# aquaskyline/Clairvoyante

Measured on AMD Instinct MI355X. Metric: candidate tensors/sec, higher is better.
Workload: dtype f32

## Files before the change

clairvoyante_amd/csrc/cv_pileup.hip:

```cpp
#include <hip/hip_runtime.h>
#include <hipcub/hipcub.hpp>

#include <cstdarg>
#include <cstdio>
#include <cstdlib>
#include <cstring>
#include <algorithm>
#include <new>
#include <string>
#include <thread>
#include <vector>

#include "../../include/clairvoyante_amd.h"
#include "cv_draw_core.hpp"

void cv_set_error(const char *fmt, ...);

#define PL_HIP(expr)                                                                              \
    do {                                                                                          \
        hipError_t _e = (expr);                                                                   \
        if (_e != hipSuccess) {                                                                   \
            cv_set_error("%s failed: %s (%s:%d)", #expr, hipGetErrorString(_e), __FILE__, __LINE__); \
            return 1;                                                                             \
        }                                                                                         \
// ... 25 lines not shown
    return ch == 'A' ? 0 : ch == 'C' ? 1 : ch == 'G' ? 2 : ch == 'T' ? 3 : -1;
}

__global__ void rebase_q0(seg_t *__restrict__ segs, int64_t n, uint32_t base)
{
    int64_t t = (int64_t)blockIdx.x * blockDim.x + threadIdx.x;
    if (t < n) segs[t].q0 += base;
}

__global__ void bucket_build(const int32_t *__restrict__ cands, int n, int32_t lo, int64_t nb,
                             int32_t *__restrict__ first)
{
    int64_t b = (int64_t)blockIdx.x * blockDim.x + threadIdx.x;
    if (b >= nb) return;
    int64_t target = (int64_t)lo + (b << BUCKET_SHIFT);
    int l = 0, h = n;
    while (l < h) {
        int m = (l + h) >> 1;
        if ((int64_t)cands[m] < target) l = m + 1; else h = m;
    }
    first[b] = l;
}

constexpr int SC_SEGS = 512;
constexpr int SC_CANDS = 40;

__global__ void __launch_bounds__(1024)
pileup_scatter(const seg_t *__restrict__ segs, int64_t nseg, const uint8_t *__restrict__ seq,
               const uint8_t *__restrict__ ref, int64_t ref_first, int64_t ref_len,
               const int32_t *__restrict__ cands, int n, const int32_t *__restrict__ bucket_first,
               int32_t bucket_lo, int64_t nb, int32_t *__restrict__ cnt, uint8_t *__restrict__ touched, int left)
{
    __shared__ int32_t tab[SC_CANDS * WIDTH * NCNT];
    const int64_t s0 = (int64_t)blockIdx.x * SC_SEGS;
    const int64_t s1 = s0 + SC_SEGS < nseg ? s0 + SC_SEGS : nseg;
    for (int k = threadIdx.x; k < SC_CANDS * WIDTH * NCNT; k += blockDim.x) tab[k] = 0;
    int i0;
    {
        const int64_t lo_c = (int64_t)segs[s0].pos - FLANK;
        int64_t b = (lo_c - bucket_lo) >> BUCKET_SHIFT;
        if (b < 0) b = 0;
        if (b >= nb) b = nb - 1;
        i0 = bucket_first[b];
        while (i0 < n && (int64_t)cands[i0] < lo_c) ++i0;
    }
    __syncthreads();
    const int lane = threadIdx.x & 63;
    const int nw = blockDim.x >> 6;
    constexpr int U = 4;
    for (int64_t sb = s0 + (threadIdx.x >> 6); sb < s1; sb += (int64_t)nw * U) {
        seg_t sg[U];
        bool on[U];
        int32_t r[U];
        int q[U], rb[U], ci[U];
#pragma unroll
        for (int u = 0; u < U; ++u) {
            const int64_t s = sb + (int64_t)u * nw;
            on[u] = s < s1;
            sg[u] = segs[on[u] ? s : s0];
        }
#pragma unroll
        for (int u = 0; u < U; ++u) {
            const int len = sg[u].info & 0xff;
            const int type = (sg[u].info >> 8) & 3;
            on[u] = on[u] && lane < len && (sg[u].info & F_CT);
            r[u] = type == T_INS ? sg[u].r0 : sg[u].r0 + lane;
            uint8_t qc = '?', rc = '?';
            if (on[u] && type != T_DEL) qc = seq[(size_t)sg[u].q0 + lane];
            const int64_t ri = (int64_t)r[u] - ref_first;
            if (on[u] && type != T_INS && ri >= 0 && ri < ref_len) rc = ref[ri];
            q[u] = base_code(qc);
            rb[u] = base_code(rc);
            int64_t b = ((int64_t)r[u] - FLANK - bucket_lo) >> BUCKET_SHIFT;
            if (b < 0) b = 0;
            if (b >= nb) on[u] = false;
            ci[u] = on[u] ? bucket_first[b] : n;
        }
#pragma unroll
        for (int u = 0; u < U; ++u) {
            if (!on[u]) continue;
            const int type = (sg[u].info >> 8) & 3;
            const int64_t lo_c = (int64_t)r[u] - FLANK, hi_c = (int64_t)r[u] + FLANK + 1;
            int i = ci[u];
            while (i < n && (int64_t)cands[i] < lo_c) ++i;
            for (; i < n; ++i) {
                const int64_t c = cands[i];
                if (c > hi_c) break;
                const int p = (int)(r[u] - c) + FLANK + 1;
                if (type != T_INS && (left || p == 0)) touched[i] = 1;
                if (!left && (int64_t)sg[u].pos > c - (FLANK + 1)) continue;
                if (p > WIDTH - 1) continue;
                int slot = -1;
                if (type == T_MATCH) {
                    if (rb[u] >= 0 && q[u] >= 0) slot = p * NCNT + 5 + q[u];
                } else if (p >= 1 && r[u] > sg[u].pos) {
                    if (type == T_DEL) {
                        if (rb[u] >= 0) slot = p * NCNT + 4;
                    } else if (q[u] >= 0) {
                        int idx = p + sg[u].adv0 + lane;
                        if (idx > WIDTH - 1 || idx < 0) idx = WIDTH - 1;
                        slot = idx * NCNT + q[u];
                    }
                }
                if (slot < 0) continue;
                const int j = i - i0;
                if (j >= 0 && j < SC_CANDS) atomicAdd(&tab[j * WIDTH * NCNT + slot], 1);
                else atomicAdd(cnt + ((size_t)i * WIDTH) * NCNT + slot, 1);
            }
        }
    }
    __syncthreads();
    const int live = n - i0 < SC_CANDS ? n - i0 : SC_CANDS;
    for (int k = threadIdx.x; k < live * WIDTH * NCNT; k += blockDim.x) {
        const int v = tab[k];
        if (v) atomicAdd(cnt + (size_t)i0 * WIDTH * NCNT + k, v);
    }
}

constexpr int EVC_SEGS = 512;
constexpr int EVC_WIN = 1536;

__global__ void __launch_bounds__(1024)
evc_count(const seg_t *__restrict__ segs, int64_t nseg, const uint8_t *__restrict__ seq, int64_t ref_first,
          int64_t ref_len, int32_t *__restrict__ pc)
{
    __shared__ int32_t tab[EVC_WIN * NPOS];
    const int64_t s0 = (int64_t)blockIdx.x * EVC_SEGS;
    const int64_t s1 = s0 + EVC_SEGS < nseg ? s0 + EVC_SEGS : nseg;
    for (int k = threadIdx.x; k < EVC_WIN * NPOS; k += blockDim.x) tab[k] = 0;
    const int64_t base = (int64_t)segs[s0].pos - 1;
    __syncthreads();
    const int lane = threadIdx.x & 63;
    for (int64_t s = s0 + (threadIdx.x >> 6); s < s1; s += (blockDim.x >> 6)) {
        const seg_t sg = segs[s];
        if (!(sg.info & F_EVC)) continue;
        const int len = sg.info & 0xff;
        const int type = (sg.info >> 8) & 3;
        int64_t r;
        int k;
        if (type == T_MATCH) {
            if (lane >= len) continue;
            const uint8_t ch = seq[(size_t)sg.q0 + lane];
            k = ch == 'A' ? 0 : ch == 'C' ? 1 : ch == 'G' ? 2 : ch == 'T' ? 3 : ch == 'N' ? 6 : -1;
            r = (int64_t)sg.r0 + lane;
        } else {
            if (lane != 0 || !(sg.info & F_FIRST)) continue;
            k = (sg.info & F_LATE) ? (type == T_INS ? 7 : 8) : (type == T_INS ? 4 : 5);
            r = (int64_t)sg.r0 - 1;
        }
        if (k < 0) continue;
        const int64_t off = r - base;
        if (off >= 0 && off < EVC_WIN) atomicAdd(&tab[off * NPOS + k], 1);
        else {
            const int64_t ri = r - ref_first;
            if (ri >= 0 && ri < ref_len) atomicAdd(pc + ri * NPOS + k, 1);
        }
    }
    __syncthreads();
    for (int k = threadIdx.x; k < EVC_WIN * NPOS; k += blockDim.x) {
        const int v = tab[k];
        if (!v) continue;
        const int64_t ri = base + k / NPOS - ref_first;
        if (ri >= 0 && ri < ref_len) atomicAdd(pc + ri * NPOS + k % NPOS, v);
    }
}

struct evc_pred {
    const int32_t *pc;
    const uint8_t *ref;
    int64_t ref_first;
    double thr, mincov;
    int has_region;
    int64_t cs, ce;
    const int64_t *bb, *be;
    int nbed;

    __device__ bool operator()(const int64_t &j) const
    {
// ... 73 lines not shown
    }
}

}

struct read_rec {
    int64_t pos;
    uint32_t seg0, nseg;
    uint8_t ct, evc, leading;
};

struct sam_part {
    std::vector<seg_t> segs;
    std::vector<uint8_t> seq;
    std::vector<read_rec> reads;
    int64_t cols = 0;
    std::string err;
};

struct dev_batch {
    seg_t *segs = nullptr;
    uint8_t *seq = nullptr;
    size_t nseg = 0, segs_cap = 0, seq_cap = 0;
};

struct cv_pileup {
    int device = 0, min_mq = 0, dcov = 250, left = 1;
    int retain = 0, evc = 0, evc_min_mq = 0, threads = 1;
    std::string contig;
    uint8_t *ref_dev = nullptr;
    int64_t ref_len = 0, ref_first = 0;
    int32_t *cand_dev = nullptr;
    int64_t n = 0;
    int32_t *bucket_dev = nullptr;
    int32_t bucket_lo = 0;
    int64_t nb = 0;
    int32_t *cnt_dev = nullptr;
    uint8_t *touched_dev = nullptr;
    int32_t *pos_cnt = nullptr;
    std::vector<sam_part> queue;
    int64_t pending_cols = 0;
    dev_batch work;
    std::vector<dev_batch> kept;
    dev_batch reserved;
    bool has_reserved = false;
    int64_t prev_pos = 0, depth_cap = 0;
    int64_t evc_prev_pos = INT64_MIN;
    int64_t evc_reads = 0;
    std::vector<int64_t> sel_host;
    std::vector<int32_t> sel_counts;
    int64_t *sel_dev = nullptr;
    int64_t nsel_dev = 0;
    bool sel_host_stale = false;
    uint8_t *cflag_dev = nullptr;
    std::vector<hipEvent_t> ev;
    std::vector<hipEvent_t> evf;
    std::vector<hipEvent_t> eve;
    float ms_scatter = 0.f, ms_final = 0.f, ms_evc = 0.f;
    int64_t cols = 0, nsegs = 0, launches = 0;
};

static int drain(std::vector<hipEvent_t> &ev, float &acc)
{
    for (size_t k = 0; k + 1 < ev.size(); k += 2) {
        float ms = 0.f;
        PL_HIP(hipEventSynchronize(ev[k + 1]));
        PL_HIP(hipEventElapsedTime(&ms, ev[k], ev[k + 1]));
        acc += ms;
        hipEventDestroy(ev[k]);
        hipEventDestroy(ev[k + 1]);
    }
    ev.clear();
    return 0;
}

struct timed {
    std::vector<hipEvent_t> &v;
// ... 13 lines not shown

extern "C" int cv_pileup_create(int device, int min_mq, int dcov, int consider_left_edge, cv_pileup **out)
{
    if (!out) { cv_set_error("cv_pileup_create: null argument"); return 1; }
    int ndev = 0;
    PL_HIP(hipGetDeviceCount(&ndev));
    if (device < 0 || device >= ndev) {
        cv_set_error("cv_pileup_create: device %d not present (%d visible)", device, ndev);
        return 1;
    }
    cv_pileup *p = new (std::nothrow) cv_pileup();
    if (!p) { cv_set_error("cv_pileup_create: out of host memory"); return 1; }
    p->device = device; p->min_mq = min_mq; p->dcov = dcov; p->left = consider_left_edge ? 1 : 0;
    *out = p;
    return 0;
}

static void free_batch(dev_batch &b)
{
    hipFree(b.segs); hipFree(b.seq);
    b = dev_batch();
}

extern "C" void cv_pileup_destroy(cv_pileup *p)
{
    if (!p) return;
    hipSetDevice(p->device);
    float sink = 0.f;
    drain(p->ev, sink); drain(p->evf, sink); drain(p->eve, sink);
    hipFree(p->ref_dev); hipFree(p->cand_dev); hipFree(p->bucket_dev); hipFree(p->cnt_dev);
    hipFree(p->touched_dev); hipFree(p->pos_cnt); hipFree(p->sel_dev); hipFree(p->cflag_dev);
    free_batch(p->work);
    if (p->has_reserved && p->retain) free_batch(p->reserved);
    for (auto &b : p->kept) free_batch(b);
    delete p;
}

extern "C" int cv_pileup_set_option(cv_pileup *p, const char *key, int64_t value)
{
    if (!p || !key) { cv_set_error("cv_pileup_set_option: null argument"); return 1; }
    if (!p->queue.empty() || p->cols) {
        cv_set_error("cv_pileup_set_option(%s): set options before the first read is added", key);
        return 1;
    }
    if (!strcmp(key, "retain")) p->retain = value != 0;
    else if (!strcmp(key, "evc")) p->evc = value != 0;
    else if (!strcmp(key, "evc_min_mq")) p->evc_min_mq = (int)value;
    else if (!strcmp(key, "threads")) p->threads = value < 1 ? 1 : value > 64 ? 64 : (int)value;
    else { cv_set_error("cv_pileup_set_option: unknown key '%s'", key); return 1; }
    return 0;
}

extern "C" int cv_pileup_set_contig(cv_pileup *p, const char *name)
{
    if (!p || !name) { cv_set_error("cv_pileup_set_contig: null argument"); return 1; }
    p->contig = name;
    return 0;
}

extern "C" int cv_pileup_set_reference(cv_pileup *p, const char *seq, int64_t len, int64_t first_pos0)
{
    if (!p || (!seq && len > 0) || len < 0) { cv_set_error("cv_pileup_set_reference: bad argument"); return 1; }
    PL_HIP(hipSetDevice(p->device));
    if (p->ref_dev) { PL_HIP(hipFree(p->ref_dev)); p->ref_dev = nullptr; }
    if (p->pos_cnt) { PL_HIP(hipFree(p->pos_cnt)); p->pos_cnt = nullptr; }
    PL_HIP(hipMalloc(&p->ref_dev, (size_t)(len > 0 ? len : 1)));
    if (len > 0) PL_HIP(hipMemcpy(p->ref_dev, seq, (size_t)len, hipMemcpyHostToDevice));
    p->ref_len = len; p->ref_first = first_pos0;
    return 0;
}

static int install_alloc(cv_pileup *p, int64_t n)
{
    hipFree(p->cand_dev); hipFree(p->bucket_dev); hipFree(p->cnt_dev); hipFree(p->touched_dev); hipFree(p->cflag_dev);
    p->cand_dev = nullptr; p->bucket_dev = nullptr; p->cnt_dev = nullptr; p->touched_dev = nullptr; p->cflag_dev = nullptr;
    p->n = n;
    size_t n1 = (size_t)(n > 0 ? n : 1);
    PL_HIP(hipMalloc(&p->cand_dev, n1 * sizeof(int32_t)));
    PL_HIP(hipMalloc(&p->cnt_dev, n1 * WIDTH * NCNT * sizeof(int32_t)));
    PL_HIP(hipMalloc(&p->touched_dev, n1));
    PL_HIP(hipMemset(p->cnt_dev, 0, n1 * WIDTH * NCNT * sizeof(int32_t)));
    PL_HIP(hipMemset(p->touched_dev, 0, n1));
    return 0;
}

static int install_buckets(cv_pileup *p, int32_t first, int32_t last)
{
    const int64_t n = p->n;
    if (n > 0) {
        p->bucket_lo = first - (FLANK + 1);
        p->nb = (((int64_t)last + FLANK + 2 - p->bucket_lo) >> BUCKET_SHIFT) + 1;
    } else {
        p->bucket_lo = 0; p->nb = 1;
    }
    PL_HIP(hipMalloc(&p->bucket_dev, (size_t)p->nb * sizeof(int32_t)));
    int threads = 256;
    bucket_build<<<(unsigned)((p->nb + threads - 1) / threads), threads>>>(p->cand_dev, (int)n, p->bucket_lo, p->nb,
                                                                             p->bucket_dev);
    PL_HIP(hipGetLastError());
    PL_HIP(hipDeviceSynchronize());
    return 0;
}

static int install_candidates(cv_pileup *p, const std::vector<int32_t> &c32)
{
    const int64_t n = (int64_t)c32.size();
    if (install_alloc(p, n)) return 1;
    if (n > 0) PL_HIP(hipMemcpy(p->cand_dev, c32.data(), (size_t)n * sizeof(int32_t), hipMemcpyHostToDevice));
    return install_buckets(p, n > 0 ? c32[0] : 0, n > 0 ? c32[(size_t)n - 1] : 0);
}

extern "C" int cv_pileup_set_candidates(cv_pileup *p, const int64_t *centers, int64_t n)
{
    if (!p || (!centers && n > 0) || n < 0) { cv_set_error("cv_pileup_set_candidates: bad argument"); return 1; }
    if (!p->queue.empty()) { cv_set_error("cv_pileup_set_candidates: reads are queued; flush first"); return 1; }
    PL_HIP(hipSetDevice(p->device));
    std::vector<int32_t> c32((size_t)n);
    for (int64_t i = 0; i < n; ++i) {
        if (centers[i] < -(1LL << 30) || centers[i] > (1LL << 31) - 64 || (i && centers[i] <= centers[i - 1])) {
            cv_set_error("cv_pileup_set_candidates: centres must be strictly ascending 1-based positions below 2^31 "
                         "(index %lld: %lld)", (long long)i, (long long)centers[i]);
            return 1;
        }
        c32[(size_t)i] = (int32_t)centers[i];
    }
    return install_candidates(p, c32);
}


static inline bool is_ws(char c) { return c == ' ' || c == '\t' || c == '\r' || c == '\v' || c == '\f'; }

static void emit(sam_part &out, int type, int flags, int64_t r0, uint64_t q0, int64_t n, int64_t pos, bool ref_advances)
{
    int64_t done = 0;
    while (done < n) {
        int64_t len = n - done < SEG_MAX ? n - done : SEG_MAX;
        seg_t s;
        s.r0 = (int32_t)(ref_advances ? r0 + done : r0);
        s.q0 = (uint32_t)(q0 + (type == T_DEL ? 0 : (uint64_t)done));
        s.info = (int32_t)len | (type << 8) | flags | (done == 0 ? F_FIRST : 0);
        s.adv0 = type == T_INS ? (int32_t)done : 0;
        s.pos = (int32_t)pos;
        out.segs.push_back(s);
        done += len;
    }
    out.cols += n;
}

static bool parse_record(const cv_pileup *p, sam_part &out, const char *line, const char *end)
// ... 268 lines not shown
    if (T == 1) {
        parse_bam_range(p, &parts[0], base, offs, 0, n, contig_ok != 0);
    } else {
        std::vector<int64_t> cut((size_t)T + 1);
        cut[0] = 0; cut[(size_t)T] = n;
        const uint64_t span = (uint64_t)(offs[n - 1] - offs[0]) + 1;
        for (int t = 1; t < T; ++t) {
            const uint32_t want = offs[0] + (uint32_t)(span * (uint64_t)t / (uint64_t)T);
            cut[(size_t)t] = std::lower_bound(offs, offs + n, want) - offs;
        }
        std::vector<std::thread> th;
        for (int t = 0; t < T; ++t)
            th.emplace_back(parse_bam_range, p, &parts[(size_t)t], base, offs, cut[(size_t)t], cut[(size_t)t + 1], contig_ok != 0);
        for (auto &x : th) x.join();
    }
    return absorb_parts(p, parts, kept);
}

extern "C" int64_t cv_pileup_pending(const cv_pileup *p) { return p ? p->pending_cols : 0; }

static int launch_scatter(cv_pileup *p, const dev_batch &b, hipStream_t st)
{
    if (p->n <= 0 || b.nseg == 0) return 0;
    if (p->ev.size() >= 128 && drain(p->ev, p->ms_scatter)) return 1;
    {
        timed t(p->ev, st);
        pileup_scatter<<<(unsigned)((b.nseg + SC_SEGS - 1) / SC_SEGS), 1024, 0, st>>>(
            b.segs, (int64_t)b.nseg, b.seq, p->ref_dev, p->ref_first, p->ref_len, p->cand_dev, (int)p->n, p->bucket_dev,
            p->bucket_lo, p->nb, p->cnt_dev, p->touched_dev, p->left);
    }
    PL_HIP(hipGetLastError());
    p->launches += 1;
    return 0;
}

extern "C" int cv_pileup_flush(cv_pileup *p, void *stream)
{
    if (!p) { cv_set_error("cv_pileup_flush: null handle"); return 1; }
    if (p->queue.empty()) return 0;
    if (!p->ref_dev || (!p->cand_dev && !p->evc)) {
        cv_set_error("cv_pileup_flush: set the reference and the candidates first");
        return 1;
    }
    PL_HIP(hipSetDevice(p->device));
    hipStream_t st = (hipStream_t)stream;
    size_t ns = 0, nq = 64;
// ... 170 lines not shown
        PL_HIP(hipMemcpy(d.bb, bb.data(), bb.size() * sizeof(int64_t), hipMemcpyHostToDevice));
        PL_HIP(hipMemcpy(d.be, be.data(), be.size() * sizeof(int64_t), hipMemcpyHostToDevice));
    }
    d.n = (int)bb.size();
    return 0;
}

struct sample_pred {
    evc_pred base;
    uint64_t seed;
    uint32_t h;
    double prob;

    __device__ bool operator()(const int64_t &j) const
    {
        if (!base(j)) return false;
        return !(cv_draw(seed, CV_DRAW_SAMPLE, h, base.ref_first + (j >> 1) + 1, (int)(j & 1)) > prob);
    }
};

template <class Pred>
static int select_entries(cv_pileup *p, const Pred &pred, hipStream_t st)
{
    hipFree(p->sel_dev); p->sel_dev = nullptr; p->nsel_dev = 0;
    const int64_t items = p->ref_len * 2;
    int64_t *count_dev = nullptr;
    PL_HIP(hipMalloc(&p->sel_dev, (size_t)items * sizeof(int64_t)));
    PL_HIP(hipMalloc(&count_dev, sizeof(int64_t)));
    int64_t nsel = 0;
    void *tmp = nullptr;
    size_t tmp_bytes = 0;
    const int64_t SLICE = 1LL << 30;
    int64_t written = 0;
    for (int64_t off = 0; off < items; off += SLICE) {
        const int cnt = (int)std::min<int64_t>(SLICE, items - off);
        hipcub::CountingInputIterator<int64_t> it(off);
        size_t need = 0;
        PL_HIP(hipcub::DeviceSelect::If(nullptr, need, it, p->sel_dev + written, count_dev, cnt, pred, st));
        if (need > tmp_bytes) { hipFree(tmp); tmp = nullptr; PL_HIP(hipMalloc(&tmp, need)); tmp_bytes = need; }
        {
            timed t(p->eve, st);
            PL_HIP(hipcub::DeviceSelect::If(tmp, need, it, p->sel_dev + written, count_dev, cnt, pred, st));
        }
        PL_HIP(hipMemcpyAsync(&nsel, count_dev, sizeof(int64_t), hipMemcpyDeviceToHost, st));
        PL_HIP(hipStreamSynchronize(st));
        written += nsel;
    }
    hipFree(tmp); hipFree(count_dev);
    int64_t *fit = nullptr;
    PL_HIP(hipMalloc(&fit, (size_t)(written > 0 ? written : 1) * sizeof(int64_t)));
    if (written) PL_HIP(hipMemcpyAsync(fit, p->sel_dev, (size_t)written * sizeof(int64_t), hipMemcpyDeviceToDevice, st));
    PL_HIP(hipStreamSynchronize(st));
    hipFree(p->sel_dev);
    p->sel_dev = fit;
    p->nsel_dev = written;
    return 0;
}

static int fetch_selected(cv_pileup *p, hipStream_t st)
{
    const int64_t written = p->nsel_dev;
    p->sel_host.resize((size_t)written);
    p->sel_counts.resize((size_t)written * 7);
    if (written) {
        int32_t *c7 = nullptr;
        PL_HIP(hipMalloc(&c7, (size_t)written * 7 * sizeof(int32_t)));
        evc_gather<<<(unsigned)((written + 255) / 256), 256, 0, st>>>(p->sel_dev, written, p->pos_cnt, c7);
        PL_HIP(hipGetLastError());
        PL_HIP(hipMemcpyAsync(p->sel_host.data(), p->sel_dev, (size_t)written * sizeof(int64_t), hipMemcpyDeviceToHost, st));
        PL_HIP(hipMemcpyAsync(p->sel_counts.data(), c7, (size_t)written * 7 * sizeof(int32_t), hipMemcpyDeviceToHost, st));
        PL_HIP(hipStreamSynchronize(st));
        hipFree(c7);
    }
    p->sel_host_stale = false;
    return 0;
}

extern "C" int cv_pileup_extract_candidates(cv_pileup *p, double threshold, double min_coverage, int has_region,
                                            int64_t ctg_start, int64_t ctg_end, const int64_t *bed_begin,
                                            const int64_t *bed_end, int64_t nbed, void *stream, int64_t *n_out)
{
    if (!p || !n_out) { cv_set_error("cv_pileup_extract_candidates: null argument"); return 1; }
    if (!p->evc) { cv_set_error("cv_pileup_extract_candidates: option 'evc' was not set"); return 1; }
    if (cv_pileup_flush(p, stream)) return 1;
    PL_HIP(hipSetDevice(p->device));
    hipStream_t st = (hipStream_t)stream;
    p->sel_host.clear(); p->sel_counts.clear();
    hipFree(p->sel_dev); p->sel_dev = nullptr; p->nsel_dev = 0; p->sel_host_stale = false;
    *n_out = 0;
    if (!p->pos_cnt || p->ref_len <= 0) return 0;
    bed_dev bed;
    if (bed_upload(bed, bed_begin, bed_end, nbed)) return 1;
    evc_pred pred{p->pos_cnt, p->ref_dev, p->ref_first, threshold, min_coverage, has_region, ctg_start, ctg_end,
                  bed.bb, bed.be, bed.n};
    if (select_entries(p, pred, st) || fetch_selected(p, st)) return 1;
    hipFree(p->sel_dev); p->sel_dev = nullptr;
    *n_out = p->nsel_dev;
    p->nsel_dev = 0;
    return 0;
}

extern "C" int cv_pileup_sample_candidates(cv_pileup *p, uint64_t seed, double output_prob, int has_region,
                                           int64_t ctg_start, int64_t ctg_end, const int64_t *bed_begin,
                                           const int64_t *bed_end, int64_t nbed, void *stream, int64_t *n_out)
{
    if (!p || !n_out) { cv_set_error("cv_pileup_sample_candidates: null argument"); return 1; }
    if (!p->evc) { cv_set_error("cv_pileup_sample_candidates: option 'evc' was not set"); return 1; }
    if (p->contig.empty()) { cv_set_error("cv_pileup_sample_candidates: no contig set (the draws are keyed by its name)"); return 1; }
    if (cv_pileup_flush(p, stream)) return 1;
    PL_HIP(hipSetDevice(p->device));
    hipStream_t st = (hipStream_t)stream;
    p->sel_host.clear(); p->sel_counts.clear();
    hipFree(p->sel_dev); p->sel_dev = nullptr; p->nsel_dev = 0; p->sel_host_stale = false;
    *n_out = 0;
    if (!p->pos_cnt || p->ref_len <= 0) return 0;
    bed_dev bed;
    if (bed_upload(bed, bed_begin, bed_end, nbed)) return 1;
    sample_pred pred{{p->pos_cnt, p->ref_dev, p->ref_first, 0.0, 0.0, has_region, ctg_start, ctg_end, bed.bb, bed.be, bed.n},
                     seed, cv_fnv1a32((const uint8_t *)p->contig.data(), (int64_t)p->contig.size()), output_prob};
    if (select_entries(p, pred, st)) return 1;
    p->sel_host_stale = true;
    *n_out = p->nsel_dev;
    return 0;
}

extern "C" int cv_pileup_get_extracted(cv_pileup *p, int64_t *pos0, int32_t *late, int32_t *counts7,
                                       int64_t info[2])
{
    if (!p) { cv_set_error("cv_pileup_get_extracted: null handle"); return 1; }
    if (p->sel_host_stale) {
        PL_HIP(hipSetDevice(p->device));
        if (fetch_selected(p, (hipStream_t)0)) return 1;
    }
    for (size_t i = 0; i < p->sel_host.size(); ++i) {
        if (pos0) pos0[i] = p->ref_first + (p->sel_host[i] >> 1);
        if (late) late[i] = (int32_t)(p->sel_host[i] & 1);
    }
    if (counts7 && !p->sel_counts.empty()) memcpy(counts7, p->sel_counts.data(), p->sel_counts.size() * sizeof(int32_t));
    if (info) { info[0] = p->evc_reads; info[1] = p->evc_prev_pos; }
    return 0;
}

extern "C" int cv_pileup_adopt_candidates(cv_pileup *p, int has_range, int64_t lo1, int64_t hi1, void *stream,
                                          int64_t *n_out)
{
    if (!p) { cv_set_error("cv_pileup_adopt_candidates: null handle"); return 1; }
    if (!p->retain) { cv_set_error("cv_pileup_adopt_candidates: option 'retain' was not set"); return 1; }
    if (cv_pileup_flush(p, stream)) return 1;
    PL_HIP(hipSetDevice(p->device));
    if (p->sel_host_stale && fetch_selected(p, (hipStream_t)stream)) return 1;
    std::vector<int32_t> c32;
    for (size_t i = 0; i < p->sel_host.size(); ++i) {
        const int64_t c = p->ref_first + (p->sel_host[i] >> 1) + 1;
        if (has_range && (c < lo1 || c > hi1)) continue;
        if (!c32.empty() && c32.back() == (int32_t)c) continue;
        c32.push_back((int32_t)c);
    }
    if (install_candidates(p, c32)) return 1;
    hipStream_t st = (hipStream_t)stream;
    for (const auto &b : p->kept) if (launch_scatter(p, b, st)) return 1;
    if (n_out) *n_out = (int64_t)c32.size();
    return 0;
}

namespace {

constexpr int32_t UNION_OUT = INT32_MAX;

__global__ void union_fill(const int64_t *__restrict__ sel, int64_t ns, int64_t ref_first, int has_range, int64_t lo1,
                           int64_t hi1, const int64_t *__restrict__ truth, int64_t nt, int32_t *__restrict__ key,
                           uint8_t *__restrict__ val)
{
    const int64_t t = (int64_t)blockIdx.x * blockDim.x + threadIdx.x;
    if (t < ns) {
        const int64_t c = ref_first + (sel[t] >> 1) + 1;
        key[t] = (has_range && (c < lo1 || c > hi1)) ? UNION_OUT : (int32_t)c;
        val[t] = CV_CENTRE_SAMPLED;
    } else if (t < ns + nt) {
        key[t] = (int32_t)truth[t - ns];
        val[t] = CV_CENTRE_TRUTH;
    }
}

__global__ void union_heads(const int32_t *__restrict__ key, int64_t m, int32_t *__restrict__ head)
// ... 16 lines not shown

struct dev_free {
    std::vector<void *> v;
    ~dev_free() { for (void *q : v) hipFree(q); }
    template <class T> hipError_t alloc(T **out, size_t bytes) { hipError_t e = hipMalloc(out, bytes ? bytes : 1); if (e == hipSuccess) v.push_back(*out); return e; }
};

}

extern "C" int cv_pileup_adopt_union(cv_pileup *p, int has_range, int64_t lo1, int64_t hi1, const int64_t *truth,
                                     int64_t ntruth, void *stream, int64_t *n_out)
{
    if (!p || ntruth < 0 || (ntruth > 0 && !truth)) { cv_set_error("cv_pileup_adopt_union: bad argument"); return 1; }
    if (!p->retain) { cv_set_error("cv_pileup_adopt_union: option 'retain' was not set"); return 1; }
    for (int64_t i = 0; i < ntruth; ++i)
        if (truth[i] < -(1LL << 30) || truth[i] > (1LL << 31) - 64 || (i && truth[i] <= truth[i - 1])) {
            cv_set_error("cv_pileup_adopt_union: truth positions must be strictly ascending 1-based positions below 2^31 "
                         "(index %lld: %lld)", (long long)i, (long long)truth[i]);
            return 1;
        }
    if (cv_pileup_flush(p, stream)) return 1;
    PL_HIP(hipSetDevice(p->device));
    hipStream_t st = (hipStream_t)stream;
    const int64_t ns = p->sel_dev ? p->nsel_dev : 0, m = ns + ntruth;
    if (m >= (1LL << 31) - 1) { cv_set_error("cv_pileup_adopt_union: %lld entries, more than one sort takes", (long long)m); return 1; }
    int64_t n = 0;
    int32_t ends[2] = {0, 0};
    dev_free tmp;
    int32_t *cands = nullptr;
    uint8_t *flags = nullptr;
    if (m > 0) {
        int64_t *truth_dev = nullptr;
        int32_t *key_in = nullptr, *key_out = nullptr, *head = nullptr, *before = nullptr;
        uint8_t *val_in = nullptr, *val_out = nullptr;
        void *ws = nullptr;
        size_t a = 0, b = 0;
        PL_HIP(hipcub::DeviceRadixSort::SortPairs(nullptr, a, (const int32_t *)nullptr, (int32_t *)nullptr, (const uint8_t *)nullptr,
                                                  (uint8_t *)nullptr, (int)m, 0, 32, st));
        PL_HIP(hipcub::DeviceScan::ExclusiveSum(nullptr, b, (const int32_t *)nullptr, (int32_t *)nullptr, (int)(m + 1), st));
        const size_t ws_bytes = a > b ? a : b;
        PL_HIP(tmp.alloc(&truth_dev, (size_t)ntruth * 8));
        PL_HIP(tmp.alloc(&key_in, (size_t)m * 4)); PL_HIP(tmp.alloc(&key_out, (size_t)m * 4));
        PL_HIP(tmp.alloc(&val_in, (size_t)m)); PL_HIP(tmp.alloc(&val_out, (size_t)m));
        PL_HIP(tmp.alloc(&head, (size_t)(m + 1) * 4)); PL_HIP(tmp.alloc(&before, (size_t)(m + 1) * 4));
        PL_HIP(tmp.alloc(&cands, (size_t)m * 4)); PL_HIP(tmp.alloc(&flags, (size_t)m));
        PL_HIP(tmp.alloc(&ws, ws_bytes));
// ... 1 lines not shown
        const unsigned grid = (unsigned)((m + 1 + 255) / 256);
        {
            timed t(p->eve, st);
            union_fill<<<grid, 256, 0, st>>>(p->sel_dev, ns, p->ref_first, has_range, lo1, hi1, truth_dev, ntruth, key_in, val_in);
            size_t wb = ws_bytes;
            PL_HIP(hipcub::DeviceRadixSort::SortPairs(ws, wb, (const int32_t *)key_in, key_out, (const uint8_t *)val_in, val_out, (int)m,
                                                      0, 32, st));
            union_heads<<<grid, 256, 0, st>>>(key_out, m, head);
            wb = ws_bytes;
            PL_HIP(hipcub::DeviceScan::ExclusiveSum(ws, wb, (const int32_t *)head, before, (int)(m + 1), st));
            union_write<<<grid, 256, 0, st>>>(key_out, val_out, head, before, m, cands, flags);
        }
        PL_HIP(hipGetLastError());
        int32_t n32 = 0;
        PL_HIP(hipMemcpyAsync(&n32, before + m, 4, hipMemcpyDeviceToHost, st));
        PL_HIP(hipStreamSynchronize(st));
        n = n32;
        if (n > 0) {
            PL_HIP(hipMemcpyAsync(&ends[0], cands, 4, hipMemcpyDeviceToHost, st));
            PL_HIP(hipMemcpyAsync(&ends[1], cands + (n - 1), 4, hipMemcpyDeviceToHost, st));
            PL_HIP(hipStreamSynchronize(st));
        }
    }
    if (install_alloc(p, n)) return 1;
    PL_HIP(hipMalloc(&p->cflag_dev, (size_t)(n > 0 ? n : 1)));
    if (n > 0) {
        PL_HIP(hipMemcpy(p->cand_dev, cands, (size_t)n * 4, hipMemcpyDeviceToDevice));
        PL_HIP(hipMemcpy(p->cflag_dev, flags, (size_t)n, hipMemcpyDeviceToDevice));
    }
    if (install_buckets(p, ends[0], ends[1])) return 1;
    for (const auto &b : p->kept) if (launch_scatter(p, b, st)) return 1;
    if (n_out) *n_out = n;
    return 0;
}

int cv_pileup_centres_dev(const cv_pileup *p, const int32_t **centres_dev, const uint8_t **flags_dev,
                                     const uint8_t **ref_dev, int64_t *ref_first, int64_t *ref_len, int64_t *n)
{
    if (!p || !centres_dev || !flags_dev || !ref_dev || !ref_first || !ref_len || !n) {
        cv_set_error("cv_pileup_centres_dev: null argument");
        return 1;
    }
    if (!p->cand_dev || !p->ref_dev) { cv_set_error("cv_pileup_centres_dev: set the reference and the candidates first"); return 1; }
    *centres_dev = p->cand_dev; *flags_dev = p->cflag_dev; *ref_dev = p->ref_dev;
    *ref_first = p->ref_first; *ref_len = p->ref_len; *n = p->n;
    return 0;
}

extern "C" int cv_pileup_recount(cv_pileup *p, void *stream)
{
    if (!p) { cv_set_error("cv_pileup_recount: null handle"); return 1; }
    if (!p->evc || !p->retain) { cv_set_error("cv_pileup_recount: needs options 'evc' and 'retain'"); return 1; }
    if (cv_pileup_flush(p, stream)) return 1;
    if (!p->pos_cnt) return 0;
    PL_HIP(hipSetDevice(p->device));
    hipStream_t st = (hipStream_t)stream;
    if (p->eve.size() >= 128 && drain(p->eve, p->ms_evc)) return 1;
    PL_HIP(hipMemsetAsync(p->pos_cnt, 0, (size_t)p->ref_len * NPOS * sizeof(int32_t), st));
    for (const auto &b : p->kept) {
        timed t(p->eve, st);
        evc_count<<<(unsigned)((b.nseg + EVC_SEGS - 1) / EVC_SEGS), 1024, 0, st>>>(b.segs, (int64_t)b.nseg, b.seq,
                                                                                   p->ref_first, p->ref_len, p->pos_cnt);
    }
    PL_HIP(hipGetLastError());
    return 0;
}

extern "C" int cv_pileup_get_candidates(cv_pileup *p, int64_t *centers, int64_t cap, int64_t *n_out)
{
    if (!p) { cv_set_error("cv_pileup_get_candidates: null handle"); return 1; }
    if (n_out) *n_out = p->n;
    if (centers && p->n > 0) {
        if (cap < p->n) { cv_set_error("cv_pileup_get_candidates: buffer holds %lld, need %lld", (long long)cap, (long long)p->n); return 1; }
        std::vector<int32_t> c32((size_t)p->n);
        PL_HIP(hipSetDevice(p->device));
        PL_HIP(hipMemcpy(c32.data(), p->cand_dev, (size_t)p->n * sizeof(int32_t), hipMemcpyDeviceToHost));
        for (int64_t i = 0; i < p->n; ++i) centers[i] = c32[(size_t)i];
    }
    return 0;
}

extern "C" int cv_pileup_finish(cv_pileup *p, float *tensors_dev, int32_t *depth_dev, uint8_t *touched_dev,
                                int subtract, void *stream)
{
    if (!p) { cv_set_error("cv_pileup_finish: null handle"); return 1; }
    if (!p->cand_dev || !p->ref_dev) {
        cv_set_error("cv_pileup_finish: set the reference and the candidates first");
        return 1;
    }
    if (cv_pileup_flush(p, stream)) return 1;
    hipStream_t st = (hipStream_t)stream;
    if (p->n == 0) return 0;
    if (tensors_dev || depth_dev) {
        timed t(p->evf, st);
        const int64_t total = p->n * WIDTH;
        pileup_finalize<<<(unsigned)((total + 255) / 256), 256, 0, st>>>(p->cnt_dev, p->cand_dev, p->n, p->ref_dev,
                                                                           p->ref_first, p->ref_len, tensors_dev,
                                                                           depth_dev, subtract);
    }
    PL_HIP(hipGetLastError());
    if (touched_dev)
        PL_HIP(hipMemcpyAsync(touched_dev, p->touched_dev, (size_t)p->n, hipMemcpyDeviceToDevice, st));
    return 0;
}

extern "C" int cv_pileup_stats(cv_pileup *p, float ms[3], int64_t counts[3])
{
    if (!p) { cv_set_error("cv_pileup_stats: null handle"); return 1; }
    PL_HIP(hipSetDevice(p->device));
    if (drain(p->ev, p->ms_scatter) || drain(p->evf, p->ms_final) || drain(p->eve, p->ms_evc)) return 1;
    if (ms) { ms[0] = p->ms_scatter; ms[1] = p->ms_final; ms[2] = p->ms_evc; }
    if (counts) { counts[0] = p->cols; counts[1] = p->nsegs; counts[2] = p->launches; }
    return 0;
}

// ... 31 lines not shown
```

Baseline: 18.77 million.

## Stage segments in LDS, ballot candidate ranges, and pool device workspaces

```diff
diff --git a/clairvoyante_amd/csrc/cv_pileup.hip b/clairvoyante_amd/csrc/cv_pileup.hip
--- a/clairvoyante_amd/csrc/cv_pileup.hip
+++ b/clairvoyante_amd/csrc/cv_pileup.hip
@@ -71,8 +71,16 @@
     first[b] = l;
 }
 
+__device__ __forceinline__ void stage_segs(seg_t *__restrict__ tile, const seg_t *__restrict__ first, int cnt)
+{
+    const int32_t *src = reinterpret_cast<const int32_t *>(first);
+    int32_t *dst = reinterpret_cast<int32_t *>(tile);
+    for (int k = threadIdx.x; k < cnt * (int)(sizeof(seg_t) / 4); k += blockDim.x) dst[k] = src[k];
+}
+
 constexpr int SC_SEGS = 512;
 constexpr int SC_CANDS = 40;
+constexpr int SC_FLIGHT = 4;
 
 __global__ void __launch_bounds__(1024)
 pileup_scatter(const seg_t *__restrict__ segs, int64_t nseg, const uint8_t *__restrict__ seq,
@@ -81,79 +89,102 @@
                int32_t bucket_lo, int64_t nb, int32_t *__restrict__ cnt, uint8_t *__restrict__ touched, int left)
 {
     __shared__ int32_t tab[SC_CANDS * WIDTH * NCNT];
+    __shared__ seg_t tile[SC_SEGS];
+    __shared__ int32_t near_c[SEG_MAX];
+    __shared__ int32_t near_touched[SC_CANDS];
     const int64_t s0 = (int64_t)blockIdx.x * SC_SEGS;
-    const int64_t s1 = s0 + SC_SEGS < nseg ? s0 + SC_SEGS : nseg;
+    const int cnt_segs = (int)((s0 + SC_SEGS < nseg ? s0 + SC_SEGS : nseg) - s0);
     for (int k = threadIdx.x; k < SC_CANDS * WIDTH * NCNT; k += blockDim.x) tab[k] = 0;
+    stage_segs(tile, segs + s0, cnt_segs);
+    const int64_t tile_lo = (int64_t)segs[s0].pos - FLANK;
     int i0;
     {
-        const int64_t lo_c = (int64_t)segs[s0].pos - FLANK;
-        int64_t b = (lo_c - bucket_lo) >> BUCKET_SHIFT;
+        int64_t b = (tile_lo - bucket_lo) >> BUCKET_SHIFT;
         if (b < 0) b = 0;
         if (b >= nb) b = nb - 1;
         i0 = bucket_first[b];
-        while (i0 < n && (int64_t)cands[i0] < lo_c) ++i0;
+        while (i0 < n && (int64_t)cands[i0] < tile_lo) ++i0;
+    }
+    if (threadIdx.x < SEG_MAX) {
+        const int j = threadIdx.x;
+        near_c[j] = j < SC_CANDS && i0 + j < n ? cands[i0 + j] : INT32_MAX;
+        if (j < SC_CANDS) near_touched[j] = 0;
     }
     __syncthreads();
     const int lane = threadIdx.x & 63;
     const int nw = blockDim.x >> 6;
-    constexpr int U = 4;
-    for (int64_t sb = s0 + (threadIdx.x >> 6); sb < s1; sb += (int64_t)nw * U) {
-        seg_t sg[U];
-        bool on[U];
-        int32_t r[U];
-        int q[U], rb[U], ci[U];
+    const int32_t my_c = near_c[lane];
+    const int64_t near_last = near_c[SC_CANDS - 1];
+    for (int sb = threadIdx.x >> 6; sb < cnt_segs; sb += nw * SC_FLIGHT) {
+        seg_t sg[SC_FLIGHT];
+        int ia[SC_FLIGHT], ib[SC_FLIGHT];
+        uint8_t qc[SC_FLIGHT], rc[SC_FLIGHT];
 #pragma unroll
-        for (int u = 0; u < U; ++u) {
-            const int64_t s = sb + (int64_t)u * nw;
-            on[u] = s < s1;
-            sg[u] = segs[on[u] ? s : s0];
-        }
-#pragma unroll
-        for (int u = 0; u < U; ++u) {
+        for (int u = 0; u < SC_FLIGHT; ++u) {
+            const int s = sb + u * nw;
+            ia[u] = ib[u] = 0;
+            qc[u] = rc[u] = '?';
+            sg[u] = tile[s < cnt_segs ? s : 0];
+            if (s >= cnt_segs || !(sg[u].info & F_CT)) continue;
             const int len = sg[u].info & 0xff;
             const int type = (sg[u].info >> 8) & 3;
-            on[u] = on[u] && lane < len && (sg[u].info & F_CT);
-            r[u] = type == T_INS ? sg[u].r0 : sg[u].r0 + lane;
-            uint8_t qc = '?', rc = '?';
-            if (on[u] && type != T_DEL) qc = seq[(size_t)sg[u].q0 + lane];
-            const int64_t ri = (int64_t)r[u] - ref_first;
-            if (on[u] && type != T_INS && ri >= 0 && ri < ref_len) rc = ref[ri];
-            q[u] = base_code(qc);
-            rb[u] = base_code(rc);
-            int64_t b = ((int64_t)r[u] - FLANK - bucket_lo) >> BUCKET_SHIFT;
-            if (b < 0) b = 0;
-            if (b >= nb) on[u] = false;
-            ci[u] = on[u] ? bucket_first[b] : n;
+            const int64_t lo_c = (int64_t)sg[u].r0 - FLANK;
+            const int64_t hi_c = (int64_t)sg[u].r0 + (type == T_INS ? 0 : len - 1) + FLANK + 1;
+            if (lo_c >= tile_lo && near_last > hi_c) {
+                const unsigned long long ge = __ballot((int64_t)my_c >= lo_c);
+                const unsigned long long le = __ballot((int64_t)my_c <= hi_c);
+                ia[u] = i0 + __ffsll((long long)ge) - 1;
+                ib[u] = i0 + __popcll(le);
+            } else {
+                int64_t b = (lo_c - bucket_lo) >> BUCKET_SHIFT;
+                if (b < 0) b = 0;
+                if (b < nb) {
+                    int i = bucket_first[b];
+                    while (i < n && (int64_t)cands[i] < lo_c) ++i;
+                    ia[u] = i; ib[u] = n;
+                }
+            }
+            if (ia[u] >= ib[u] || lane >= len) continue;
+            if (type != T_DEL) qc[u] = seq[(size_t)sg[u].q0 + lane];
+            const int64_t ri = (int64_t)sg[u].r0 + lane - ref_first;
+            if (type != T_INS && ri >= 0 && ri < ref_len) rc[u] = ref[ri];
         }
 #pragma unroll
-        for (int u = 0; u < U; ++u) {
-            if (!on[u]) continue;
+        for (int u = 0; u < SC_FLIGHT; ++u) {
+            if (ia[u] >= ib[u]) continue;
+            const int len = sg[u].info & 0xff;
             const int type = (sg[u].info >> 8) & 3;
-            const int64_t lo_c = (int64_t)r[u] - FLANK, hi_c = (int64_t)r[u] + FLANK + 1;
-            int i = ci[u];
-            while (i < n && (int64_t)cands[i] < lo_c) ++i;
-            for (; i < n; ++i) {
-                const int64_t c = cands[i];
+            const bool on = lane < len;
+            const int32_t r = type == T_INS ? sg[u].r0 : sg[u].r0 + lane;
+            const int64_t hi_c = (int64_t)sg[u].r0 + (type == T_INS ? 0 : len - 1) + FLANK + 1;
+            const int q = base_code(qc[u]), rb = base_code(rc[u]);
+            for (int i = ia[u]; i < ib[u]; ++i) {
+                const int j = i - i0;
+                const bool near = j >= 0 && j < SC_CANDS;
+                const int64_t c = near ? near_c[j] : cands[i];
                 if (c > hi_c) break;
-                const int p = (int)(r[u] - c) + FLANK + 1;
-                if (type != T_INS && (left || p == 0)) touched[i] = 1;
+                const int64_t pw = (int64_t)r - c + FLANK + 1;
+                const bool hit = on && pw >= 0 && pw <= WIDTH;
+                const bool mark = hit && type != T_INS && (left || pw == 0);
+                if (near) { if (mark) near_touched[j] = 1; }
+                else if (__ballot(mark)) { if (lane == 0) touched[i] = 1; }
                 if (!left && (int64_t)sg[u].pos > c - (FLANK + 1)) continue;
-                if (p > WIDTH - 1) continue;
+                if (!hit || pw > WIDTH - 1) continue;
+                const int p = (int)pw;
                 int slot = -1;
                 if (type == T_MATCH) {
-                    if (rb[u] >= 0 && q[u] >= 0) slot = p * NCNT + 5 + q[u];
-                } else if (p >= 1 && r[u] > sg[u].pos) {
+                    if (rb >= 0 && q >= 0) slot = p * NCNT + 5 + q;
+                } else if (p >= 1 && r > sg[u].pos) {
                     if (type == T_DEL) {
-                        if (rb[u] >= 0) slot = p * NCNT + 4;
-                    } else if (q[u] >= 0) {
+                        if (rb >= 0) slot = p * NCNT + 4;
+                    } else if (q >= 0) {
                         int idx = p + sg[u].adv0 + lane;
                         if (idx > WIDTH - 1 || idx < 0) idx = WIDTH - 1;
-                        slot = idx * NCNT + q[u];
+                        slot = idx * NCNT + q;
                     }
                 }
                 if (slot < 0) continue;
-                const int j = i - i0;
-                if (j >= 0 && j < SC_CANDS) atomicAdd(&tab[j * WIDTH * NCNT + slot], 1);
+                if (near) atomicAdd(&tab[j * WIDTH * NCNT + slot], 1);
                 else atomicAdd(cnt + ((size_t)i * WIDTH) * NCNT + slot, 1);
             }
         }
@@ -164,45 +195,60 @@
         const int v = tab[k];
         if (v) atomicAdd(cnt + (size_t)i0 * WIDTH * NCNT + k, v);
     }
+    if ((int)threadIdx.x < live && near_touched[threadIdx.x]) touched[i0 + threadIdx.x] = 1;
 }
 
 constexpr int EVC_SEGS = 512;
 constexpr int EVC_WIN = 1536;
+constexpr int EVC_FLIGHT = 4;
 
 __global__ void __launch_bounds__(1024)
 evc_count(const seg_t *__restrict__ segs, int64_t nseg, const uint8_t *__restrict__ seq, int64_t ref_first,
           int64_t ref_len, int32_t *__restrict__ pc)
 {
     __shared__ int32_t tab[EVC_WIN * NPOS];
+    __shared__ seg_t tile[EVC_SEGS];
     const int64_t s0 = (int64_t)blockIdx.x * EVC_SEGS;
-    const int64_t s1 = s0 + EVC_SEGS < nseg ? s0 + EVC_SEGS : nseg;
+    const int cnt_segs = (int)((s0 + EVC_SEGS < nseg ? s0 + EVC_SEGS : nseg) - s0);
     for (int k = threadIdx.x; k < EVC_WIN * NPOS; k += blockDim.x) tab[k] = 0;
-    const int64_t base = (int64_t)segs[s0].pos - 1;
+    stage_segs(tile, segs + s0, cnt_segs);
     __syncthreads();
+    const int64_t base = (int64_t)tile[0].pos - 1;
     const int lane = threadIdx.x & 63;
-    for (int64_t s = s0 + (threadIdx.x >> 6); s < s1; s += (blockDim.x >> 6)) {
-        const seg_t sg = segs[s];
-        if (!(sg.info & F_EVC)) continue;
-        const int len = sg.info & 0xff;
-        const int type = (sg.info >> 8) & 3;
-        int64_t r;
-        int k;
-        if (type == T_MATCH) {
-            if (lane >= len) continue;
-            const uint8_t ch = seq[(size_t)sg.q0 + lane];
-            k = ch == 'A' ? 0 : ch == 'C' ? 1 : ch == 'G' ? 2 : ch == 'T' ? 3 : ch == 'N' ? 6 : -1;
-            r = (int64_t)sg.r0 + lane;
-        } else {
-            if (lane != 0 || !(sg.info & F_FIRST)) continue;
-            k = (sg.info & F_LATE) ? (type == T_INS ? 7 : 8) : (type == T_INS ? 4 : 5);
-            r = (int64_t)sg.r0 - 1;
-        }
-        if (k < 0) continue;
-        const int64_t off = r - base;
-        if (off >= 0 && off < EVC_WIN) atomicAdd(&tab[off * NPOS + k], 1);
-        else {
-            const int64_t ri = r - ref_first;
-            if (ri >= 0 && ri < ref_len) atomicAdd(pc + ri * NPOS + k, 1);
+    const int nw = blockDim.x >> 6;
+    for (int sb = threadIdx.x >> 6; sb < cnt_segs; sb += nw * EVC_FLIGHT) {
+        int64_t r[EVC_FLIGHT];
+        int k[EVC_FLIGHT];
+        uint8_t ch[EVC_FLIGHT];
+#pragma unroll
+        for (int u = 0; u < EVC_FLIGHT; ++u) {
+            const int s = sb + u * nw;
+            r[u] = 0; k[u] = -1; ch[u] = 0;
+            const seg_t sg = tile[s < cnt_segs ? s : 0];
+            if (s >= cnt_segs || !(sg.info & F_EVC)) continue;
+            const int len = sg.info & 0xff;
+            const int type = (sg.info >> 8) & 3;
+            if (type == T_MATCH) {
+                if (lane >= len) continue;
+                ch[u] = seq[(size_t)sg.q0 + lane];
+                k[u] = -2;
+                r[u] = (int64_t)sg.r0 + lane;
+            } else if (lane == 0 && (sg.info & F_FIRST)) {
+                k[u] = (sg.info & F_LATE) ? (type == T_INS ? 7 : 8) : (type == T_INS ? 4 : 5);
+                r[u] = (int64_t)sg.r0 - 1;
+            }
+        }
+#pragma unroll
+        for (int u = 0; u < EVC_FLIGHT; ++u) {
+            int kk = k[u];
+            if (kk == -2) kk = ch[u] == 'A' ? 0 : ch[u] == 'C' ? 1 : ch[u] == 'G' ? 2 : ch[u] == 'T' ? 3 : ch[u] == 'N' ? 6 : -1;
+            if (kk < 0) continue;
+            const int64_t off = r[u] - base;
+            if (off >= 0 && off < EVC_WIN) atomicAdd(&tab[off * NPOS + kk], 1);
+            else {
+                const int64_t ri = r[u] - ref_first;
+                if (ri >= 0 && ri < ref_len) atomicAdd(pc + ri * NPOS + kk, 1);
+            }
         }
     }
     __syncthreads();
@@ -322,6 +368,11 @@
     seg_t *segs = nullptr;
     uint8_t *seq = nullptr;
     size_t nseg = 0, segs_cap = 0, seq_cap = 0;
+};
+
+struct dev_buf {
+    void *ptr = nullptr;
+    size_t cap = 0;
 };
 
 struct cv_pileup {
@@ -353,6 +404,11 @@
     int64_t nsel_dev = 0;
     bool sel_host_stale = false;
     uint8_t *cflag_dev = nullptr;
+    dev_buf ws_sel, ws_select_tmp, ws_count, ws_gather, ws_cand, ws_cnt, ws_touched, ws_cflag, ws_bucket;
+    hipStream_t ws_stream = nullptr;
+    bool ws_used = false;
+    std::vector<int32_t> cand_host;
+    bool cand_host_valid = false;
     std::vector<hipEvent_t> ev;
     std::vector<hipEvent_t> evf;
     std::vector<hipEvent_t> eve;
@@ -412,14 +468,34 @@
     b = dev_batch();
 }
 
+static int ws_room(dev_buf &b, size_t bytes)
+{
+    if (bytes == 0) bytes = 1;
+    if (b.ptr && bytes <= b.cap && bytes >= b.cap / 4) return 0;
+    hipFree(b.ptr);
+    b.ptr = nullptr; b.cap = 0;
+    PL_HIP(hipMalloc(&b.ptr, bytes));
+    b.cap = bytes;
+    return 0;
+}
+
+static int ws_enter(cv_pileup *p, hipStream_t st)
+{
+    if (p->ws_used && p->ws_stream != st) PL_HIP(hipDeviceSynchronize());
+    p->ws_stream = st; p->ws_used = true;
+    return 0;
+}
+
 extern "C" void cv_pileup_destroy(cv_pileup *p)
 {
     if (!p) return;
     hipSetDevice(p->device);
     float sink = 0.f;
     drain(p->ev, sink); drain(p->evf, sink); drain(p->eve, sink);
-    hipFree(p->ref_dev); hipFree(p->cand_dev); hipFree(p->bucket_dev); hipFree(p->cnt_dev);
-    hipFree(p->touched_dev); hipFree(p->pos_cnt); hipFree(p->sel_dev); hipFree(p->cflag_dev);
+    hipFree(p->ref_dev); hipFree(p->pos_cnt);
+    for (dev_buf *b : {&p->ws_sel, &p->ws_select_tmp, &p->ws_count, &p->ws_gather, &p->ws_cand, &p->ws_cnt, &p->ws_touched,
+                       &p->ws_cflag, &p->ws_bucket})
+        hipFree(b->ptr);
     free_batch(p->work);
     if (p->has_reserved && p->retain) free_batch(p->reserved);
     for (auto &b : p->kept) free_batch(b);
@@ -460,21 +536,21 @@
     return 0;
 }
 
-static int install_alloc(cv_pileup *p, int64_t n)
-{
-    hipFree(p->cand_dev); hipFree(p->bucket_dev); hipFree(p->cnt_dev); hipFree(p->touched_dev); hipFree(p->cflag_dev);
-    p->cand_dev = nullptr; p->bucket_dev = nullptr; p->cnt_dev = nullptr; p->touched_dev = nullptr; p->cflag_dev = nullptr;
+static int install_alloc(cv_pileup *p, int64_t n, hipStream_t st)
+{
+    if (ws_enter(p, st)) return 1;
     p->n = n;
-    size_t n1 = (size_t)(n > 0 ? n : 1);
-    PL_HIP(hipMalloc(&p->cand_dev, n1 * sizeof(int32_t)));
-    PL_HIP(hipMalloc(&p->cnt_dev, n1 * WIDTH * NCNT * sizeof(int32_t)));
-    PL_HIP(hipMalloc(&p->touched_dev, n1));
-    PL_HIP(hipMemset(p->cnt_dev, 0, n1 * WIDTH * NCNT * sizeof(int32_t)));
-    PL_HIP(hipMemset(p->touched_dev, 0, n1));
-    return 0;
-}
-
-static int install_buckets(cv_pileup *p, int32_t first, int32_t last)
+    p->cflag_dev = nullptr; p->cand_host_valid = false;
+    const size_t n1 = (size_t)(n > 0 ? n : 1);
+    if (ws_room(p->ws_cand, n1 * sizeof(int32_t)) || ws_room(p->ws_cnt, n1 * WIDTH * NCNT * sizeof(int32_t)) ||
+        ws_room(p->ws_touched, n1)) return 1;
+    p->cand_dev = (int32_t *)p->ws_cand.ptr; p->cnt_dev = (int32_t *)p->ws_cnt.ptr; p->touched_dev = (uint8_t *)p->ws_touched.ptr;
+    PL_HIP(hipMemsetAsync(p->cnt_dev, 0, n1 * WIDTH * NCNT * sizeof(int32_t), st));
+    PL_HIP(hipMemsetAsync(p->touched_dev, 0, n1, st));
+    return 0;
+}
+
+static int install_buckets(cv_pileup *p, int32_t first, int32_t last, hipStream_t st)
 {
     const int64_t n = p->n;
     if (n > 0) {
@@ -483,21 +559,26 @@
     } else {
         p->bucket_lo = 0; p->nb = 1;
     }
-    PL_HIP(hipMalloc(&p->bucket_dev, (size_t)p->nb * sizeof(int32_t)));
+    if (ws_room(p->ws_bucket, (size_t)p->nb * sizeof(int32_t))) return 1;
+    p->bucket_dev = (int32_t *)p->ws_bucket.ptr;
     int threads = 256;
-    bucket_build<<<(unsigned)((p->nb + threads - 1) / threads), threads>>>(p->cand_dev, (int)n, p->bucket_lo, p->nb,
-                                                                             p->bucket_dev);
+    bucket_build<<<(unsigned)((p->nb + threads - 1) / threads), threads, 0, st>>>(p->cand_dev, (int)n, p->bucket_lo, p->nb,
+                                                                                    p->bucket_dev);
     PL_HIP(hipGetLastError());
-    PL_HIP(hipDeviceSynchronize());
-    return 0;
-}
-
-static int install_candidates(cv_pileup *p, const std::vector<int32_t> &c32)
+    return 0;
+}
+
+static int install_candidates(cv_pileup *p, std::vector<int32_t> &c32, hipStream_t st)
 {
     const int64_t n = (int64_t)c32.size();
-    if (install_alloc(p, n)) return 1;
-    if (n > 0) PL_HIP(hipMemcpy(p->cand_dev, c32.data(), (size_t)n * sizeof(int32_t), hipMemcpyHostToDevice));
-    return install_buckets(p, n > 0 ? c32[0] : 0, n > 0 ? c32[(size_t)n - 1] : 0);
+    if (install_alloc(p, n, st)) return 1;
+    p->cand_host.swap(c32);
+    p->cand_host_valid = true;
+    if (n > 0) {
+        PL_HIP(hipMemcpyAsync(p->cand_dev, p->cand_host.data(), (size_t)n * sizeof(int32_t), hipMemcpyHostToDevice, st));
+        PL_HIP(hipStreamSynchronize(st));
+    }
+    return install_buckets(p, n > 0 ? p->cand_host[0] : 0, n > 0 ? p->cand_host[(size_t)n - 1] : 0, st);
 }
 
 extern "C" int cv_pileup_set_candidates(cv_pileup *p, const int64_t *centers, int64_t n)
@@ -514,7 +595,7 @@
         }
         c32[(size_t)i] = (int32_t)centers[i];
     }
-    return install_candidates(p, c32);
+    return install_candidates(p, c32, (hipStream_t)0);
 }
 
 
@@ -829,6 +910,7 @@
 static int launch_scatter(cv_pileup *p, const dev_batch &b, hipStream_t st)
 {
     if (p->n <= 0 || b.nseg == 0) return 0;
+    if (ws_enter(p, st)) return 1;
     if (p->ev.size() >= 128 && drain(p->ev, p->ms_scatter)) return 1;
     {
         timed t(p->ev, st);
@@ -1045,37 +1127,28 @@
 template <class Pred>
 static int select_entries(cv_pileup *p, const Pred &pred, hipStream_t st)
 {
-    hipFree(p->sel_dev); p->sel_dev = nullptr; p->nsel_dev = 0;
+    p->sel_dev = nullptr; p->nsel_dev = 0;
     const int64_t items = p->ref_len * 2;
-    int64_t *count_dev = nullptr;
-    PL_HIP(hipMalloc(&p->sel_dev, (size_t)items * sizeof(int64_t)));
-    PL_HIP(hipMalloc(&count_dev, sizeof(int64_t)));
+    if (ws_enter(p, st) || ws_room(p->ws_sel, (size_t)items * sizeof(int64_t)) || ws_room(p->ws_count, sizeof(int64_t))) return 1;
+    int64_t *sel = (int64_t *)p->ws_sel.ptr, *count_dev = (int64_t *)p->ws_count.ptr;
     int64_t nsel = 0;
-    void *tmp = nullptr;
-    size_t tmp_bytes = 0;
     const int64_t SLICE = 1LL << 30;
     int64_t written = 0;
     for (int64_t off = 0; off < items; off += SLICE) {
         const int cnt = (int)std::min<int64_t>(SLICE, items - off);
         hipcub::CountingInputIterator<int64_t> it(off);
         size_t need = 0;
-        PL_HIP(hipcub::DeviceSelect::If(nullptr, need, it, p->sel_dev + written, count_dev, cnt, pred, st));
-        if (need > tmp_bytes) { hipFree(tmp); tmp = nullptr; PL_HIP(hipMalloc(&tmp, need)); tmp_bytes = need; }
+        PL_HIP(hipcub::DeviceSelect::If(nullptr, need, it, sel + written, count_dev, cnt, pred, st));
+        if (ws_room(p->ws_select_tmp, need)) return 1;
         {
             timed t(p->eve, st);
-            PL_HIP(hipcub::DeviceSelect::If(tmp, need, it, p->sel_dev + written, count_dev, cnt, pred, st));
+            PL_HIP(hipcub::DeviceSelect::If(p->ws_select_tmp.ptr, need, it, sel + written, count_dev, cnt, pred, st));
         }
         PL_HIP(hipMemcpyAsync(&nsel, count_dev, sizeof(int64_t), hipMemcpyDeviceToHost, st));
         PL_HIP(hipStreamSynchronize(st));
         written += nsel;
     }
-    hipFree(tmp); hipFree(count_dev);
-    int64_t *fit = nullptr;
-    PL_HIP(hipMalloc(&fit, (size_t)(written > 0 ? written : 1) * sizeof(int64_t)));
-    if (written) PL_HIP(hipMemcpyAsync(fit, p->sel_dev, (size_t)written * sizeof(int64_t), hipMemcpyDeviceToDevice, st));
-    PL_HIP(hipStreamSynchronize(st));
-    hipFree(p->sel_dev);
-    p->sel_dev = fit;
+    p->sel_dev = sel;
     p->nsel_dev = written;
     return 0;
 }
@@ -1086,14 +1159,13 @@
     p->sel_host.resize((size_t)written);
     p->sel_counts.resize((size_t)written * 7);
     if (written) {
-        int32_t *c7 = nullptr;
-        PL_HIP(hipMalloc(&c7, (size_t)written * 7 * sizeof(int32_t)));
+        if (ws_enter(p, st) || ws_room(p->ws_gather, (size_t)written * 7 * sizeof(int32_t))) return 1;
+        int32_t *c7 = (int32_t *)p->ws_gather.ptr;
         evc_gather<<<(unsigned)((written + 255) / 256), 256, 0, st>>>(p->sel_dev, written, p->pos_cnt, c7);
         PL_HIP(hipGetLastError());
         PL_HIP(hipMemcpyAsync(p->sel_host.data(), p->sel_dev, (size_t)written * sizeof(int64_t), hipMemcpyDeviceToHost, st));
         PL_HIP(hipMemcpyAsync(p->sel_counts.data(), c7, (size_t)written * 7 * sizeof(int32_t), hipMemcpyDeviceToHost, st));
         PL_HIP(hipStreamSynchronize(st));
-        hipFree(c7);
     }
     p->sel_host_stale = false;
     return 0;
@@ -1109,7 +1181,7 @@
     PL_HIP(hipSetDevice(p->device));
     hipStream_t st = (hipStream_t)stream;
     p->sel_host.clear(); p->sel_counts.clear();
-    hipFree(p->sel_dev); p->sel_dev = nullptr; p->nsel_dev = 0; p->sel_host_stale = false;
+    p->sel_dev = nullptr; p->nsel_dev = 0; p->sel_host_stale = false;
     *n_out = 0;
     if (!p->pos_cnt || p->ref_len <= 0) return 0;
     bed_dev bed;
@@ -1117,7 +1189,7 @@
     evc_pred pred{p->pos_cnt, p->ref_dev, p->ref_first, threshold, min_coverage, has_region, ctg_start, ctg_end,
                   bed.bb, bed.be, bed.n};
     if (select_entries(p, pred, st) || fetch_selected(p, st)) return 1;
-    hipFree(p->sel_dev); p->sel_dev = nullptr;
+    p->sel_dev = nullptr;
     *n_out = p->nsel_dev;
     p->nsel_dev = 0;
     return 0;
@@ -1134,7 +1206,7 @@
     PL_HIP(hipSetDevice(p->device));
     hipStream_t st = (hipStream_t)stream;
     p->sel_host.clear(); p->sel_counts.clear();
-    hipFree(p->sel_dev); p->sel_dev = nullptr; p->nsel_dev = 0; p->sel_host_stale = false;
+    p->sel_dev = nullptr; p->nsel_dev = 0; p->sel_host_stale = false;
     *n_out = 0;
     if (!p->pos_cnt || p->ref_len <= 0) return 0;
     bed_dev bed;
@@ -1179,10 +1251,10 @@
         if (!c32.empty() && c32.back() == (int32_t)c) continue;
         c32.push_back((int32_t)c);
     }
-    if (install_candidates(p, c32)) return 1;
     hipStream_t st = (hipStream_t)stream;
+    if (install_candidates(p, c32, st)) return 1;
     for (const auto &b : p->kept) if (launch_scatter(p, b, st)) return 1;
-    if (n_out) *n_out = (int64_t)c32.size();
+    if (n_out) *n_out = p->n;
     return 0;
 }
 
@@ -1245,6 +1317,7 @@
     if (cv_pileup_flush(p, stream)) return 1;
     PL_HIP(hipSetDevice(p->device));
     hipStream_t st = (hipStream_t)stream;
+    if (ws_enter(p, st)) return 1;
     const int64_t ns = p->sel_dev ? p->nsel_dev : 0, m = ns + ntruth;
     if (m >= (1LL << 31) - 1) { cv_set_error("cv_pileup_adopt_union: %lld entries, more than one sort takes", (long long)m); return 1; }
     int64_t n = 0;
@@ -1292,13 +1365,13 @@
             PL_HIP(hipStreamSynchronize(st));
         }
     }
-    if (install_alloc(p, n)) return 1;
-    PL_HIP(hipMalloc(&p->cflag_dev, (size_t)(n > 0 ? n : 1)));
+    if (install_alloc(p, n, st) || ws_room(p->ws_cflag, (size_t)n)) return 1;
+    p->cflag_dev = (uint8_t *)p->ws_cflag.ptr;
     if (n > 0) {
-        PL_HIP(hipMemcpy(p->cand_dev, cands, (size_t)n * 4, hipMemcpyDeviceToDevice));
-        PL_HIP(hipMemcpy(p->cflag_dev, flags, (size_t)n, hipMemcpyDeviceToDevice));
-    }
-    if (install_buckets(p, ends[0], ends[1])) return 1;
+        PL_HIP(hipMemcpyAsync(p->cand_dev, cands, (size_t)n * 4, hipMemcpyDeviceToDevice, st));
+        PL_HIP(hipMemcpyAsync(p->cflag_dev, flags, (size_t)n, hipMemcpyDeviceToDevice, st));
+    }
+    if (install_buckets(p, ends[0], ends[1], st)) return 1;
     for (const auto &b : p->kept) if (launch_scatter(p, b, st)) return 1;
     if (n_out) *n_out = n;
     return 0;
@@ -1342,10 +1415,13 @@
     if (n_out) *n_out = p->n;
     if (centers && p->n > 0) {
         if (cap < p->n) { cv_set_error("cv_pileup_get_candidates: buffer holds %lld, need %lld", (long long)cap, (long long)p->n); return 1; }
-        std::vector<int32_t> c32((size_t)p->n);
-        PL_HIP(hipSetDevice(p->device));
-        PL_HIP(hipMemcpy(c32.data(), p->cand_dev, (size_t)p->n * sizeof(int32_t), hipMemcpyDeviceToHost));
-        for (int64_t i = 0; i < p->n; ++i) centers[i] = c32[(size_t)i];
+        if (!p->cand_host_valid) {
+            p->cand_host.resize((size_t)p->n);
+            PL_HIP(hipSetDevice(p->device));
+            PL_HIP(hipMemcpy(p->cand_host.data(), p->cand_dev, (size_t)p->n * sizeof(int32_t), hipMemcpyDeviceToHost));
+            p->cand_host_valid = true;
+        }
+        for (int64_t i = 0; i < p->n; ++i) centers[i] = p->cand_host[(size_t)i];
     }
     return 0;
 }
@@ -1361,6 +1437,7 @@
     if (cv_pileup_flush(p, stream)) return 1;
     hipStream_t st = (hipStream_t)stream;
     if (p->n == 0) return 0;
+    if (ws_enter(p, st)) return 1;
     if (tensors_dev || depth_dev) {
         timed t(p->evf, st);
         const int64_t total = p->n * WIDTH;
```

After: 18.77 million, median of 2. About the same (+0.0%).
